# tesseract-robotics/trajopt

Hardware: AMD Instinct MI355X
Metric: SQP iters/s (+ QP solves/s), 7-DOF x 30-wp x 1024-batch glass_upright (higher is better)
Workload: dtype f64; 1 GPU; config 1: glass_upright 7-DOF 30-waypoint, collision cost, batch=1024 random seeds per GPU; n_dof=7, n_steps=30, batch_per_gpu=1024, qp_n=572, qp_m=876, parallelism=seeds sharded, dp1

## Files before the change

### trajopt_amd/csrc/tmx_api.cpp

```cpp
#include <algorithm>
#include <cstddef>
#include <limits>
#include <string>
#include <vector>

#include "tmx_kernels.h"
#include "tmx_wave_kernels.h"
#include "tmx_wave_plan.h"

#ifdef TMX_HOST_EMU
#include <chrono>
thread_local tmx_emu_idx tmx_emu_threadIdx, tmx_emu_blockIdx, tmx_emu_blockDim, tmx_emu_gridDim;
thread_local double* tmx_emu_smem = nullptr;
double tmx_emu_now_ms()
{
  return std::chrono::duration<double, std::milli>(std::chrono::steady_clock::now().time_since_epoch()).count();
}
#else
#include <rccl/rccl.h>
#endif

#define HIPCHK(call)                                                                                                  \
  do                                                                                                                  \
  {                                                                                                                   \
// ... 1528 lines not shown
    int n_coll = 0;
    for (int k : kind)
      n_coll += (k == SLOT_COLLISION || k == SLOT_COLLISION_LVS) ? 1 : 0;
    const char* force = std::getenv("TMX_FORCE_COMPACT");
    const bool on = (force && force[0] == '1') || (!(force && force[0] == '0') && (R >= 1024 || R2 > 0) && 2 * n_coll > R);
    if (on)
      P.coef_far |= 2;
  }
  if (dyn_p && !qp_dense)
    P.coef_far |= 4;
  P.dbg_flags = 0;
  P.wave_ok = 0;
  P.wv_gmax = 2;
  P.wv_aux2 = 0;
  P.wv_plan = nullptr;
  P.row_perm = nullptr;
  {
    const char* env = std::getenv("TMX_ROW_PERM");
    const int NT = TMX_QP_NT;
    if (!(env && env[0] == '0') && R <= 2 * NT && TMX_QP_NT == 256)
    {
      std::vector<int> perm(2 * (size_t)NT, -1), cheap, heavy;
      for (int r = 0; r < R; ++r)
        (naux[r] > 1 ? heavy : cheap).push_back(r);
      const int extra = std::max(0, R - NT), two_first = NT - extra;
      const int prot_first = extra > 0 ? (two_first / 64) * 64 : NT;
      std::vector<int> pool(cheap);
      pool.insert(pool.end(), heavy.begin(), heavy.end());
      size_t take = 0;
      for (int q = 0; q < 2; ++q)
        for (int i = 0; i < extra; ++i)
          perm[(size_t)q * NT + two_first + i] = pool[take++];
      for (int tdx = prot_first; tdx < two_first && take < pool.size(); ++tdx)
        perm[tdx] = pool[take++];
      const int n_free = std::min(prot_first, two_first);
      const size_t n_cheap_left = take < cheap.size() ? cheap.size() - take : 0, n_left = pool.size() - take, n_heavy_left = n_left - n_cheap_left;
      if ((int)n_left > n_free)
        perm.clear();
      else
      {
        for (size_t i = 0; i < n_cheap_left; ++i)
          perm[i] = pool[take + i];
        for (size_t i = 0; i < n_heavy_left; ++i)
          perm[(size_t)n_free - n_heavy_left + i] = pool[take + n_cheap_left + i];
      }
      if (!perm.empty())
      {
        tmx_status rcp;
        if ((rcp = upload(ctx, ctx->prob_allocs, &P.row_perm, perm)) != TMX_OK)
          return rcp;
      }
    }
  }
#if TMX_IS_DEVICE
  {
    const char* env = std::getenv("TMX_WAVE");
    const bool allowed = env && env[0] == '1';
    std::vector<int> plan(TMX_WV_NT * TMX_WV_REC, 0);
    int gmax = 4, aux2 = 0, n3 = 0;
    if (allowed && P.flavor == 0 && R2 == 0 && P.coef_far == 0 && !qp_dense && !P.st && !P.band && !P.use_time && P.n_fx == 0 &&
        wave_plan_build(D, T, R, st.data(), naux.data(), plan.data(), &gmax, &aux2, &n3))
    {
      const size_t small_ints_w = 2 * (size_t)(P.n_max + 1) + 4 * (size_t)R + 2 + 16 + 16 + 512;
      size_t small = std::max<size_t>((tmx_eval_scratch_doubles(R, D * T, (int)vel_first.size(), n_costs, n_cnts) + n_costs + n_cnts + 8) * sizeof(double),
                                      small_ints_w * sizeof(int) + 64);
      small = std::max<size_t>(small, tmx_cvx_scratch_doubles(P.n_cp, D) * sizeof(double));
      const size_t lds = std::max(small, wave_lds_doubles(D, T, R) * sizeof(double));
      if (lds <= 40 * 1024)
      {
        tmx_status rcw;
        if ((rcw = upload(ctx, ctx->prob_allocs, &P.wv_plan, plan)) != TMX_OK)
          return rcw;
        P.wave_ok = 1;
        P.wv_gmax = gmax;
        P.wv_aux2 = aux2;
        ctx->smem_wave = lds;
      }
    }
  }
#endif
  ctx->smem_qp = qp_smem_bytes(D, T, R, NA, R2, P.coef_far);
  ctx->tt_scratch = 0;
  if (P.tt_chain > 0 || P.tv_chain)
  {
    const size_t tt_bytes = ((P.tv_chain ? qp_tv_doubles(D, T) : qp_tt_doubles(D, T, P.tt_chain)) + 2) * sizeof(double);
    const char* force = std::getenv("TMX_TT_PLACE");
    if (TMX_QP_COLD_IN_LDS && !(force && force[0] == '2') && (ctx->smem_qp > 160 * 1024 || ctx->smem_qp + tt_bytes <= 160 * 1024))
    {
      P.tt_place = 1;
      ctx->smem_qp += tt_bytes;
    }
    else
    {
      P.tt_place = 2;
      ctx->tt_scratch = tt_bytes / sizeof(double);
    }
  }
  if (!ctx->dp)
  {
    void* p = nullptr;
    HIPCHK(hipMalloc(&p, sizeof(DevProblem)));
    ctx->dp = static_cast<DevProblem*>(p);
  }
  HIPCHK(hipMemcpy(ctx->dp, &P, sizeof(DevProblem), hipMemcpyHostToDevice));
  if (std::getenv("TMX_VERBOSE"))
    std::fprintf(stderr, "[tmx] QP engine: %s; TotalTime terms %d, as rank-one terms on the block chain %d; squared velocity-with-time cost instances %d, "
// ... 1374 lines not shown
{
  if (!ctx || !a || !b || !out || n < 1 || op < 0 || op > 2)
    return TMX_ERR_INVALID;
  HIPCHK(hipSetDevice(ctx->device));
  std::vector<void*> pool;
  double *da = nullptr, *db = nullptr, *dout = nullptr;
  tmx_status rc;
  if ((rc = dalloc(ctx, pool, &da, (size_t)n)) != TMX_OK || (rc = dalloc(ctx, pool, &db, (size_t)n)) != TMX_OK ||
      (rc = dalloc(ctx, pool, &dout, (size_t)n)) != TMX_OK)
  {
    free_pool(pool);
    return rc;
  }
  hipError_t e = hipMemcpy(da, a, sizeof(double) * n, hipMemcpyHostToDevice);
  if (e == hipSuccess)
    e = hipMemcpy(db, b, sizeof(double) * n, hipMemcpyHostToDevice);
  if (e == hipSuccess)
  {
    TMX_LAUNCH(k_detmath, 64, 256, 0, ctx->stream, op, n, da, db, dout);
    e = hipStreamSynchronize(ctx->stream);
  }
  if (e == hipSuccess)
    e = hipMemcpy(out, dout, sizeof(double) * n, hipMemcpyDeviceToHost);
  free_pool(pool);
  if (e != hipSuccess)
  {
    ctx->err = std::string("tmx_debug_detmath: ") + hipGetErrorString(e);
    return TMX_ERR_DEVICE;
  }
  return TMX_OK;
}

__attribute__((visibility("default"))) tmx_status tmx_debug_admm_iters(tmx_ctx* ctx, int64_t* out)
{
  if (!ctx || !out || ctx->hb.B <= 0)
    return TMX_ERR_INVALID;
  static_assert(sizeof(long long) == sizeof(int64_t), "");
  if (hipMemcpy(out, ctx->hb.admm_iters, sizeof(int64_t) * ctx->hb.B, hipMemcpyDeviceToHost) != hipSuccess)
    return TMX_ERR_DEVICE;
  return TMX_OK;
}

__attribute__((visibility("default"))) tmx_status tmx_debug_set_flags(tmx_ctx* ctx, int flags)
{
  if (!ctx || !ctx->have_problem || !ctx->dp)
    return TMX_ERR_INVALID;
  TMX_REFUSE_WHILE_PENDING(ctx);
  HIPCHK(hipSetDevice(ctx->device));
  ctx->hp.dbg_flags = flags;
  HIPCHK(hipMemcpy(reinterpret_cast<char*>(ctx->dp) + offsetof(DevProblem, dbg_flags), &flags, sizeof(int), hipMemcpyHostToDevice));
  return TMX_OK;
}

__attribute__((visibility("default"))) tmx_status tmx_debug_set_fused(tmx_ctx* ctx, int mode)
{
  if (!ctx || mode < 0 || mode > 2)
    return TMX_ERR_INVALID;
  ctx->mode = mode;
  return TMX_OK;
}

tmx_status tmx_kernel_stats_reset(tmx_ctx* ctx)
{
  if (!ctx)
    return TMX_ERR_INVALID;
  ctx->ms_admm = ctx->ms_convexify = ctx->ms_evaluate = 0.0;
  ctx->launches_admm = 0;
  return TMX_OK;
}
}
```

### trajopt_amd/csrc/tmx_solve.h

```cpp
#pragma once
#include "tmx_qp.h"
#include "tmx_terms.h"

#if TMX_IS_DEVICE
#define TMX_ATOMIC_ADD_U64(ptr, v) atomicAdd((unsigned long long*)(ptr), (unsigned long long)(v))
#else
#define TMX_ATOMIC_ADD_U64(ptr, v) __atomic_fetch_add((unsigned long long*)(ptr), (unsigned long long)(v), __ATOMIC_RELAXED)
#endif

TMX_DEVFN double aux_cost(const DevProblem* P, const double* merit, int r)
{
  if (P->flavor == 1)
  {
    const double cf = (P->slot_kind[r] == SLOT_COLLISION_LVS) ? P->slot_objc[r] : P->slot_scale[r];
    return (P->slot_iscnt[r] ? merit[P->slot_owner[r]] : 1.0) * cf;
  }
  return P->slot_iscnt[r] ? merit[P->slot_owner[r]] : P->slot_objc[r];
}
TMX_DEVFN double primary_q(const DevProblem* P, const double* qdyn, int v)
{
  if (P->flavor == 1)
    return (fabs(qdyn[v]) < 1e-7) ? 0.0 : qdyn[v];
  return P->pq[v];
}

TMX_DEVFN double aux_sign(int naux, int k) { return (naux == 1) ? -1.0 : (k == 0 ? 1.0 : -1.0); }

struct CscOut
{
  long long *P_p, *P_i, *A_p, *A_i;
  double *P_x, *q, *A_x, *l, *u;
};

TMX_DEVFN double tv_p_val(const DevProblem* P, const double* tv_aff, int sgm, int jj, int ia, int ib, bool& any)
{
  double v = 0.0;
  any = false;
  if (tv_aff == nullptr || sgm < 0 || sgm >= P->T - 1)
    return v;
  for (int c = 0; c < P->n_tv; ++c)
    if ((jj < 0 || P->tv_joint[c] == jj) && sgm >= P->tv_first[c] && sgm < P->tv_last[c])
    {
      const double* rec = tv_aff + ((size_t)c * P->T + sgm) * TMX_TV_REC;
      for (int half = 0; half < 2; ++half)
      {
        const double ca = half ? -rec[ia] : rec[ia], cb = half ? -rec[ib] : rec[ib];
        const double coeff = ((ia == ib) ? ca * ca : 2 * ca * cb) * P->tv_coeff[c];
        if (coeff != 0.0)
        {
          v += (ia == ib) ? 2.0 * coeff : coeff;
          any = true;
        }
      }
    }
// ... 882 lines not shown
#ifdef TMX_PROFILE
#define TMX_PROF_ENTER(sh)                                                                                            \
  long long pc[16] = { 0, 0, 0, 0, 0, 0, 0, 0, 0, 0, 0, 0, 0, 0, 0, 0 };                                             \
  long long tlast = TMX_CLK()
#define TMX_PROF_LEAVE(sh)                                                                                            \
  do                                                                                                                  \
  {                                                                                                                   \
    if (threadIdx.x == TMX_PROF_TID)                                                                                  \
      for (int q_ = 0; q_ < 16; ++q_)                                                                                 \
      {                                                                                                               \
        Bt->prof[(size_t)b * 16 + q_] += pc[q_];                                                                      \
        pc[q_] = 0;                                                                                                   \
      }                                                                                                               \
  } while (0)
#else
#define TMX_PROF_ENTER(sh)                                                                                            \
  long long pc[16];                                                                                                   \
  long long tlast = 0;                                                                                                \
  (void)pc;                                                                                                           \
  (void)tlast
#define TMX_PROF_LEAVE(sh) ((void)0)
#endif
TMX_DEVFN QpShared* qp_ws_rebuild(QpWs& w, const DevProblem* P, const DevBatch* Bt, int b, double* smem)
{
  const int D = P->D, T = P->T, R = P->R;
  double* scratch = Bt->qp_scratch + (size_t)b * Bt->qp_scratch_stride;
#if TMX_QP_COLD_IN_LDS
  qp_ws_carve(w, smem, smem + qp_lds_doubles(D, T, R, P->NA, P->n_link), scratch, D, T, R, P->NA, P->n_link, P->coef_far);
#else
  qp_ws_carve(w, smem, scratch + qp_far_doubles(D, T, R, P->NA, P->n_link, P->coef_far), scratch, D, T, R, P->NA, P->n_link, P->coef_far);
#endif
#if TMX_LINK_ROWS
  w.c2i = P->slot_c2;
#endif
  DPart dpt;
  dpart_make(T, dpt);
  qp_ws_alias_deltas(w, P, dpt);
  QpShared* sh = reinterpret_cast<QpShared*>(w.wself);
  w.rho = sh->rho;
  w.sigma = sh->sigma;
  w.alpha = sh->alpha;
  w.c = sh->c;
  w.cinv = sh->cinv;
  return sh;
}
static_assert(sizeof(QpShared) <= sizeof(QpWs), "QpShared must fit the descriptor slot");
template <class T>
TMX_DEVFN T* tmx_uniform_ptr(T* p)
{
  const unsigned long long v = (unsigned long long)p;
  const unsigned lo = __builtin_amdgcn_readfirstlane((unsigned)v), hi = __builtin_amdgcn_readfirstlane((unsigned)(v >> 32));
  return (T*)(((unsigned long long)hi << 32) | lo);
}
__device__ __attribute__((noinline)) static int qp_check_nl(const DevProblem* P_in, const DevBatch* Bt_in, int b_in, int iter_in, unsigned lds_in)
{
  const DevProblem* P = tmx_uniform_ptr(P_in);
  const DevBatch* Bt = tmx_uniform_ptr(Bt_in);
  const int b = __builtin_amdgcn_readfirstlane(b_in), iter = __builtin_amdgcn_readfirstlane(iter_in);
  const int tid = threadIdx.x, NT = TMX_QP_NT;
  double* smem = (double*)(tmx_lds_d*)(size_t)(unsigned)__builtin_amdgcn_readfirstlane((int)lds_in);
  const tmx_osqp_settings& st = P->osqp;
  QpWs w;
  QpShared* sh = qp_ws_rebuild(w, P, Bt, b, smem);
  QpInfo info = sh->info;
  TMX_PROF_ENTER(sh);
  const bool can_check = st.check_termination && (iter % st.check_termination == 0);
  const bool do_rho = st.adaptive_rho && st.adaptive_rho_interval && (iter % st.adaptive_rho_interval == 0);
  int ended = 0;
  if (can_check || do_rho)
  {
    info.iter = iter;
    if (sh->have_res)
    {
      const double* m = sh->res;
      info.prim_res = m[0];
      info.dual_res = w.cinv * m[6];
      info.s_prim = m[1];
      info.s_z = m[2];
      info.s_ax = m[3];
      info.u_z = m[4];
      info.u_ax = m[5];
      info.s_dual = m[7];
      info.s_q = m[8];
      info.s_aty = m[9];
      info.s_px = m[10];
      info.u_q = m[11];
      info.u_aty = m[12];
      info.u_px = m[13];
    }
    else
      compute_residuals(w, P, w.xp, w.xa, w.yr, w.ybp, w.yba, 0, info, info.prim_res, info.dual_res, true, tid, NT);
    TMX_TICK(6);
  }
  if (can_check && TMX_UNI_B(check_termination(w, P, info, false, tid, NT)))
    ended = 1;
  TMX_TICK(3);
  double rho = w.rho;
  if (!ended && do_rho)
  {
    const double rho_new = rho_estimate(w, info);
    if (TMX_UNI_B((rho_new > w.rho * st.adaptive_rho_tolerance) || (rho_new < w.rho / st.adaptive_rho_tolerance)))
    {
      w.rho = fmin(fmax(rho_new, TMX_RHO_MIN), TMX_RHO_MAX);
      rho = w.rho;
      info.rho_updates += 1;
      TMX_TICK(6);
// ... 223 lines not shown
    sh->can_check = can_check ? 1 : 0;
    sh->iter = iter;
#ifdef TMX_PROFILE
    for (int q_ = 0; q_ < 16; ++q_)
      Bt->prof[(size_t)b * 16 + q_] += pc[q_];
#endif
  }
  TMX_SYNC();
}
#endif

template <bool HBM = false, bool BANDK = true, bool ROWSK = true>
TMX_DEVFN void qp_solve_block(const DevProblem* P, const DevBatch* Bt, int b, double* smem, int tid, int NT, double* chain_lds = nullptr)
{
  const int D = P->D, T = P->T, NX = P->NX, R = P->R;
  const tmx_osqp_settings& st = P->osqp;
  QpWs w;
  {
    double* scratch = Bt->qp_scratch + (size_t)b * Bt->qp_scratch_stride;
#if TMX_QP_COLD_IN_LDS
    qp_ws_carve(w, smem, smem + qp_lds_doubles(D, T, R, P->NA, P->n_link), scratch, D, T, R, P->NA, P->n_link, P->coef_far);
#else
    qp_ws_carve(w, smem, scratch + qp_far_doubles(D, T, R, P->NA, P->n_link, P->coef_far), scratch, D, T, R, P->NA, P->n_link, P->coef_far);
#endif
    if (chain_lds)
      qp_ws_chain_to_lds(w, chain_lds);
  }
  if constexpr (BANDK)
    qp_ws_attach_band(w, P->band, Bt->band_ws + (size_t)b * (size_t)Bt->band_stride, (ROWSK && P->band_rows) ? P->n_link : 0);
  [[maybe_unused]] const double* dyn_H = nullptr;
  [[maybe_unused]] const double* dyn_g = nullptr;
  if constexpr (ROWSK)
    if (P->coef_far & 4)
    {
      w.pb = Bt->qp_scratch + (size_t)b * Bt->qp_scratch_stride + qp_dynp_offset(D, T, R, P->NA, P->n_link, P->coef_far);
      dyn_H = Bt->fx_H + (size_t)b * P->n_fx_cost * D * D;
      dyn_g = Bt->fx_g + (size_t)b * P->n_fx_cost * D;
    }
  if constexpr (ROWSK)
    if (P->tt_chain > 0 || P->tv_chain)
      qp_ws_attach_tt(w, P, smem, Bt->qp_scratch + (size_t)b * Bt->qp_scratch_stride);
  long long pc[16] = { 0, 0, 0, 0, 0, 0, 0, 0, 0, 0, 0, 0, 0, 0, 0, 0 };
  long long tlast = TMX_CLK();
  const int* g_act = Bt->active + (size_t)b * R;
  const double* g_coef = Bt->coef + (size_t)b * R * D;
  const double* g_rhs = Bt->rhs + (size_t)b * R;
  [[maybe_unused]] const double* g_coef2 = Bt->coef2 + (size_t)b * P->n_link * D;
  const double* g_x = Bt->x + (size_t)b * NX;
  const double* g_merit = Bt->merit + (size_t)b * P->n_cnts;
  const double trust = Bt->trust[b];
  const int* dims = Bt->dims + 4 * b;
  const unsigned long long* hs = Bt->hashes + 4 * b;

  for (int r = tid; r < R; r += NT)
  {
    w.act[r] = g_act[r];
    w.naux[r] = P->slot_naux[r];
    w.aoff[r] = P->slot_aoff[r];
    w.slot_t[r] = P->slot_t[r];
    w.wp_list[r] = P->wp_list[r];
    w.flg_r[r] = 0;
    w.Er[r] = 1.0;
    w.zr[r] = 0.0;
    w.yr[r] = 0.0;
    w.dyr[r] = 0.0;
    w.lor[r] = P->slot_eq[r] ? g_rhs[r] : -TMX_OSQP_INFTY;
    w.hir[r] = g_rhs[r];
    if (g_act[r] || w.c_alist == nullptr)
    {
      for (int j = 0; j < D; ++j)
        w.coef[r * D + j] = g_act[r] ? g_coef[r * D + j] : 0.0;
#if TMX_LINK_ROWS
      if (P->n_link > 0 && P->slot_c2[r] >= 0)
        for (int j = 0; j < D; ++j)
          w.c2[P->slot_c2[r] * D + j] = g_act[r] ? g_coef2[P->slot_c2[r] * D + j] : 0.0;
#endif
    }
#if TMX_LINK_ROWS
    if (w.band_rows && P->slot_c2[r] >= 0)
    {
      const int ci = P->slot_c2[r];
      const int ord = slot_is_diff(P->slot_kind[r]) ? diff_row_order(P, r) : 1;
      ws_fo(w)[ci] = ord >= 2 ? (ord << 8 | P->slot_sub[r]) : 0;
      ws_cf(w)[2 * ci] = (ord >= 2 && g_act[r]) ? diff_row_coef(P, r, 2) : 0.0;
      ws_cf(w)[2 * ci + 1] = (ord >= 3 && g_act[r]) ? diff_row_coef(P, r, 3) : 0.0;
    }
#endif
    const double oc = aux_cost(P, g_merit, r);
    for (int k = 0; k < P->slot_naux[r]; ++k)
    {
      const int a = P->slot_aoff[r] + k;
      w.sa[a] = aux_sign(P->slot_naux[r], k);
      w.qa[a] = oc;
      w.bba[a] = 1.0;
      w.Da[a] = 1.0;
      w.Eba[a] = 1.0;
      w.xa[a] = 0.0;
      w.zba[a] = 0.0;
      w.yba[a] = 0.0;
      w.dxa[a] = 0.0;
      w.dyba[a] = 0.0;
      w.flg_ba[a] = 0;
    }
  }
  for (int v = tid; v < NX; v += NT)
  {
    const int j = v % D;
    const double xi = fmin(fmax(g_x[v], P->jl[j]), P->ju[j]);
    const double lb = fmax(xi - trust, P->jl[j]), ub = fmin(xi + trust, P->ju[j]);
// ... 52 lines not shown
        bool any;
        double va = 0.0, vc = 0.0;
        if (j < D - 1)
        {
          w.pd[v] = P->pd[v] + tv_p_diag(P, aff, t, j, any);
          if (v < NX - D)
          {
            w.po[v] = P->po[v] + tv_p_val(P, aff, t, j, 0, 1, any);
            vc = tv_p_val(P, aff, t, j, 0, 2, any);
          }
          if (t >= 1)
            va = tv_p_val(P, aff, t - 1, j, 1, 2, any);
        }
        else if (t >= 1)
          w.pd[v] = P->pd[v] + tv_p_val(P, aff, t - 1, -1, 2, 2, any);
        ws_tva(w)[v] = va;
        ws_tvc(w)[v] = vc;
        w.qp[v] = tv_q_lin(P, aff, t, j, w.qp[v]);
      }
    if (w.band)
    {
      w.po2[v] = (v < NX - 2 * D) ? P->po2[v] : 0.0;
      w.po3[v] = (v < NX - 3 * D) ? P->po3[v] : 0.0;
    }
    w.bbp[v] = 1.0;
    w.Dp[v] = 1.0;
    w.Ebp[v] = 1.0;
    w.xp[v] = 0.0;
    w.zbp[v] = 0.0;
    w.ybp[v] = 0.0;
    w.dxp[v] = 0.0;
    w.dybp[v] = 0.0;
    w.flg_bp[v] = 0;
  }
  if constexpr (ROWSK)
    if (w.pb != nullptr)
      for (int e = tid; e < T * D * D; e += NT)
      {
        const int t = e / (D * D), i = (e / D) % D, j = e % D;
        double v = 0.0;
        if (i != j)
          for (int c = 0; c < P->n_fx; ++c)
            if (fx_is_quad(P->fx_kind[c]) && P->fx_t[c] == t)
            {
              const double h = dyn_H[(size_t)P->fx_ci[c] * D * D + (i < j ? i : j) * D + (i < j ? j : i)];
              if (h != 0.0)
                v += h;
            }
        w.pb[e] = v;
      }
  for (int t = tid; t <= T; t += NT)
  {
    w.wp_start[t] = P->wp_start[t];
    int acc = 0;
    for (int u = 0; u < t; ++u)
    {
      const int c = P->wp_start[u + 1] - P->wp_start[u];
      acc += c + (c & 1);
    }
    w.wp_pst[t] = acc;
    for (int u = P->wp_start[t]; t < T && u < P->wp_start[t + 1]; ++u)
      w.row_epos[P->wp_list[u]] = acc + (u - P->wp_start[t]);
  }
#if TMX_LINK_ROWS
  w.c2i = P->slot_c2;
#endif
  w.sigma = st.sigma;
  w.alpha = st.alpha;
  w.c = 1.0;
  w.cinv = 1.0;
  TMX_SYNC();
  {
    int* scan = reinterpret_cast<int*>(w.red);
    const int C = (R + NT - 1) / NT;
    const int r0 = tid * C < R ? tid * C : R, r1 = (tid + 1) * C < R ? (tid + 1) * C : R;
    for (int pass = 0; pass < 2; ++pass)
    {
      int cnt = 0;
      for (int r = r0; r < r1; ++r)
        cnt += w.act[r] ? (pass == 0 ? 1 : w.naux[r]) : 0;
      TMX_SYNC();
      scan[tid] = cnt;
      TMX_SYNC();
      int off = 0;
      for (int u = 0; u < tid; ++u)
        off += scan[u];
      for (int r = r0; r < r1; ++r)
      {
        if (pass == 0)
          w.row_ref[r] = off;
        else
          w.aux_ref[r] = NX + off;
        off += w.act[r] ? (pass == 0 ? 1 : w.naux[r]) : 0;
      }
    }
    TMX_SYNC();
    rows_compact_build(w, P, scan, tid, NT);
  }
  const int n = dims[0], m = dims[1], mg = m - n;
  DPart dpt;
  dpart_make(T, dpt);
  const bool lds_tmp = (w.G != nullptr) && ((size_t)NX + 3 * (size_t)P->NA <= (size_t)dpt.P * w.Gn * w.Gs);
  double* const t_ebp = lds_tmp ? w.G : w.dybp;
  double* const t_eba = lds_tmp ? w.G + NX : w.dyba;
  double* const t_da = lds_tmp ? w.G + NX + P->NA : w.ta;
  double* const acc_da = lds_tmp ? w.G + NX + 2 * P->NA : w.Da;
  if (lds_tmp)
  {
    for (int a = tid; a < P->NA; a += NT)
      acc_da[a] = 1.0;
    TMX_SYNC();
  }

#if defined(TMX_FINE) && TMX_FINE == 4
  TMX_TICK(13);
#endif
  for (int it = 0; it < st.scaling; ++it)
  {
    for (int v = tid; v < NX; v += NT)
    {
      const int t = v / D, j = v % D;
      double cn = fabs(w.pd[v]);
      if (t > 0)
        cn = fmax(cn, fabs(w.po[v - D]));
      if (t < T - 1)
        cn = fmax(cn, fabs(w.po[v]));
      if (w.band)
        cn = fmax(cn, band_col_norm(w, v));
      if (w.pb != nullptr)
        for (int i = 0; i < D; ++i)
          cn = fmax(cn, fabs(w.pb[(size_t)t * D * D + i * D + j]));
      if (w.tvo != 0)
        cn = fmax(cn, tv_p_col_norm(w, v));
      {
        const int q1 = w.wl_start[t + 1];
        int q = w.wl_start[t];
        for (; q + 4 <= q1; q += 4)
        {
          const int r0 = w.wl_list[q], r1 = w.wl_list[q + 1], r2 = w.wl_list[q + 2], r3 = w.wl_list[q + 3];
          const int a0 = w.act[r0], a1 = w.act[r1], a2 = w.act[r2], a3 = w.act[r3];
          const double c0 = w.coef[r0 * D + j], c1 = w.coef[r1 * D + j], c2 = w.coef[r2 * D + j], c3 = w.coef[r3 * D + j];
          cn = a0 ? fmax(cn, fabs(c0)) : cn;
          cn = a1 ? fmax(cn, fabs(c1)) : cn;
          cn = a2 ? fmax(cn, fabs(c2)) : cn;
          cn = a3 ? fmax(cn, fabs(c3)) : cn;
        }
        for (; q < q1; ++q)
        {
          const int r = w.wl_list[q];
          if (w.act[r])
            cn = fmax(cn, fabs(w.coef[r * D + j]));
        }
      }
#if TMX_LINK_ROWS
      if (w.n_link > 0 && t > 0)
        for (int q = w.wl_start[t - 1]; q < w.wl_start[t]; ++q)
        {
          const int r = w.wl_list[q];
          if (w.act[r] && w.c2i[r] >= 0)
            cn = fmax(cn, fabs(w.c2[w.c2i[r] * D + j]));
        }
      if (w.band_rows)
        for (int k = 2; k <= 3 && k <= t; ++k)
          for (int q = w.wl_start[t - k]; q < w.wl_start[t - k + 1]; ++q)
          {
            const int r = w.wl_list[q];
            const int ci = w.c2i[r];
            if (!w.act[r] || ci < 0)
              continue;
// ... 161 lines not shown
      c_temp = limit_scaling(c_temp);
      w.red[128] = 1.0 / c_temp;
    }
    TMX_SYNC();
    const double ct = w.red[128];
    for (int v = tid; v < NX; v += NT)
    {
      w.pd[v] *= ct;
      w.po[v] *= ct;
      if (w.band)
      {
        w.po2[v] *= ct;
        w.po3[v] *= ct;
      }
      w.qp[v] *= ct;
    }
    if (w.pb != nullptr)
      for (int e = tid; e < T * D * D; e += NT)
        w.pb[e] *= ct;
    if (w.ttn > 0 && tid == 0)
      for (int k = 0; k < w.ttn; ++k)
        ws_ttw(w)[k] *= ct;
    if (w.tvo != 0)
      for (int v = tid; v < 2 * NX; v += NT)
        ws_tva(w)[v] *= ct;
    TMX_ROWS(w, r)
      if (w.act[r])
        for (int k = 0; k < w.naux[r]; ++k)
          w.qa[w.aoff[r] + k] *= ct;
    w.c *= ct;
    TMX_SYNC();
  }
  w.cinv = 1.0 / w.c;
  if (lds_tmp)
    for (int a = tid; a < P->NA; a += NT)
      w.Da[a] = acc_da[a];
  for (int v = tid; v < NX; v += NT)
  {
    w.lbp[v] *= w.Ebp[v];
    w.ubp[v] *= w.Ebp[v];
    w.typ_bp[v] = constr_type(w.lbp[v], w.ubp[v]);
  }
  TMX_ROWS(w, r)
  {
    if (!w.act[r])
      continue;
    w.lor[r] *= w.Er[r];
    w.hir[r] *= w.Er[r];
    w.typ_r[r] = constr_type(w.lor[r], w.hir[r]);
    for (int k = 0; k < w.naux[r]; ++k)
      w.typ_ba[w.aoff[r] + k] = constr_type(0.0, TMX_OSQP_INFTY * w.Eba[w.aoff[r] + k]);
  }
  TMX_SYNC();

#if defined(TMX_FINE) && TMX_FINE == 4
  TMX_TICK(15);
#endif
  const int* pd4 = Bt->prev_dims + 4 * b;
  const unsigned long long* pws = Bt->prev_ws + 2 * b;
  bool warm = Bt->prev_ok[b] && st.warm_starting;
  const bool P_eq = warm && pd4[0] == dims[0] && pd4[2] == dims[2] && pws[0] == hs[2];
  const bool A_eq = P_eq && pd4[0] == dims[0] && pd4[1] == dims[1] && pd4[3] == dims[3] && pws[1] == hs[3];
  warm = TMX_UNI_B(warm && P_eq && A_eq);
#if defined(TMX_HOST_EMU) && !defined(TMX_EMU_SIMT)
  if (const char* fq = std::getenv("TMX_EMU_FAULT_WARM_QP"))
    if (Bt->rec_count[b] >= std::atoi(fq) && warm)
      warm = false;
#endif
  if (P->flavor == 1)
  {
    warm = TMX_UNI_B(st.warm_starting != 0);
    w.rho = Bt->prev_ok[b] ? Bt->prev_rho[b] : st.rho;
  }
  else
    w.rho = warm ? Bt->prev_rho[b] : st.rho;
  w.rho = fmin(fmax(w.rho, TMX_RHO_MIN), TMX_RHO_MAX);
  if (warm)
  {
    const double* xq = Bt->xq + (size_t)b * P->n_max;
    const double* yq = Bt->yq + (size_t)b * P->m_max;
    for (int v = tid; v < NX; v += NT)
    {
      w.xp[v] = (1.0 / w.Dp[v]) * xq[v];
      w.ybp[v] = ((1.0 / w.Ebp[v]) * yq[mg + v]) * w.c;
    }
    TMX_ROWS(w, r)
      if (w.act[r])
      {
        w.yr[r] = ((1.0 / w.Er[r]) * yq[w.row_ref[r]]) * w.c;
        for (int k = 0; k < w.naux[r]; ++k)
        {
          const int a = w.aoff[r] + k;
          w.xa[a] = (1.0 / w.Da[a]) * xq[w.aux_ref[r] + k];
          w.yba[a] = ((1.0 / w.Eba[a]) * yq[mg + w.aux_ref[r] + k]) * w.c;
        }
      }
    TMX_SYNC();
    for (int v = tid; v < NX; v += NT)
      w.zbp[v] = w.bbp[v] * w.xp[v];
    TMX_ROWS(w, r)
      if (w.act[r])
      {
        const int t = w.slot_t[r];
        double ax = 0.0;
        for (int j = 0; j < D; ++j)
          ax += w.coef[r * D + j] * w.xp[t * D + j];
#if TMX_LINK_ROWS
        ax += link_dot(w, r, t, w.xp);
#endif
        for (int k = 0; k < w.naux[r]; ++k)
        {
          const int a = w.aoff[r] + k;
          ax += w.sa[a] * w.xa[a];
          w.zba[a] = w.bba[a] * w.xa[a];
        }
        w.zr[r] = ax;
      }
    TMX_SYNC();
  }

  TMX_TICK(0);
#if TMX_IS_DEVICE
  const bool fast = TMX_UNI_B(!HBM && (NT == TMX_QP_NT) && (R <= 512) && dpart_supported(w, NT) && !TMX_HAS_PAIRS(w) && w.c_alist == nullptr && w.band == 0 && w.pb == nullptr && w.ttn == 0 && w.tvo == 0 && TMX_FAST_ALLOWED);
#else
  const bool fast = false;
#endif
#if TMX_IS_DEVICE
  if (fast)
    qp_ws_alias_deltas(w, P, dpt);
#endif
  kkt_factor(w, P, 0, w.sigma, st.delta, tid, NT);
  kkt_invert(w, fast, tid, NT, pc, tlast);
  if (w.ttn > 0)
    tt_factor(w, tid, NT);
  admm_cache_weights(w, tid, NT);
  TMX_TICK(15);
  QpInfo info;
  info.status = 11;
  info.iter = 0;
  info.rho_updates = 0;
  info.polish_status = 0;
  info.prim_res = info.dual_res = 0.0;
  int iter = 0;
  bool can_check = false, terminated = false;
#if TMX_ADMM_OUTLINED
  if (fast)
  {
    QpShared* sh = reinterpret_cast<QpShared*>(w.wself);
    if (tid == 0)
    {
      sh->rho = w.rho;
      sh->sigma = w.sigma;
      sh->alpha = w.alpha;
      sh->c = w.c;
      sh->cinv = w.cinv;
      sh->info = info;
      sh->terminated = 0;
      sh->can_check = 0;
      sh->iter = 0;
      sh->have_res = 0;
    }
    TMX_SYNC();
    {
      unsigned lds_off = (unsigned)(size_t)smem;
      TMX_ASM_OPAQUE_SGPR(lds_off);
      qp_admm_fast_nl(P, Bt, b, lds_off);
    }
#ifdef TMX_PROFILE
    tlast = TMX_CLK();
#endif
    info = sh->info;
    w.rho = sh->rho;
    terminated = sh->terminated != 0;
    can_check = sh->can_check != 0;
    iter = sh->iter;
    TMX_SYNC();
  }
  else
#endif
// ... 1234 lines not shown
```

### trajopt_amd/csrc/tmx_types.h

```cpp
#pragma once
#include "../../include/tmx.h"
#include "tmx_platform.h"

enum
{
  SLOT_FIXED = 0,
  SLOT_CARTPOSE = 1,
  SLOT_JOINTPOS = 2,
  SLOT_COLLISION = 3,
  SLOT_JOINTPOS_INEQ = 4,
  SLOT_JOINTVEL = 5,
  SLOT_JOINTVEL_INEQ = 6,
  SLOT_COLLISION_LVS = 7,
  SLOT_FUNC = 9,
  SLOT_CARTVEL = 8,
  SLOT_JOINTVEL_TIME = 10,
  SLOT_TOTAL_TIME = 11
};
#ifndef TMX_LINK_ROWS
#define TMX_LINK_ROWS 1
#endif

enum
{
// ... 23 lines not shown
  int *wp_list;
  double *pd, *po, *pq;
  int *p_colptr;
  int *vel_first, *vel_last, *vel_cost, *vel_kind;
  double *vel_coeffs, *vel_targets;
  int *cp_t, *cp_owner, *cp_iscnt, *cp_nrows, *cp_idx, *cp_slot0;
  double *cp_coeff, *cp_target;
  int *ls_link;
  double *ls_center, *ls_radius, *ob_center, *ob_radius;
  int *own_lo, *own_hi;
  int coef_far;
  double *ob_axis;
  int *slot_c2;
  int n_link;
  int *slot_sub3;
  double *slot_aux3;
  int lvs_kmax;
  int flavor;
  int n_sq;
  double *po2, *po3;
  int n_stencil;
  int qp_dense;
  int st;
  int n_fx, n_fx_cost;
  int *fx_t, *fx_kind, *fx_owner, *fx_op0, *fx_nops, *fx_c0, *fx_nout, *fx_slot0, *fx_ci;
  int *fx_ops;
  double *fx_consts;
  double *ls_axis;
  int n_ls_capsule;
  double *ob_box;
  int n_ob_box;
  double *mesh;
  int band;
  int band_rows;
  int* ls_hull;
  double* hull;
  int n_ls_hull;
  int DK;
  int use_time;
  int n_tv;
  int *tv_owner, *tv_joint, *tv_first, *tv_last;
  double *tv_coeff, *tv_target, *tv_up, *tv_lo;
  int n_tt;
  int *tt_owner, *tt_form, *tt_slot;
  double *tt_coeff, *tt_limit;
  int wave_ok;
  int wv_gmax;
  int wv_aux2;
  int* wv_plan;
  int* row_perm;
  int dbg_flags;
  int tt_chain, tt_place;
  int tv_chain;
};
TMX_HOSTDEVFN int slot_is_diff(int kind) { return kind == SLOT_JOINTVEL || kind == SLOT_JOINTVEL_INEQ; }
#define TMX_TV_REC 5
TMX_HOSTDEVFN int fx_is_quad(int kind) { return kind == 0 || kind == 1 || kind == 3; }
TMX_HOSTDEVFN int fx_is_rows(int kind) { return kind == 2 || kind == 4; }

struct DevBatch
{
  int B, max_rec;
  double *x0, *x, *xnew;
  double *cost_vals, *cnt_viols, *new_cost_vals, *new_cnt_viols, *merit;
  double *trust, *total_cost, *prev_rho;
  int *phase, *iter, *merit_inc, *qp_fail, *status, *retval, *n_fe, *n_qp, *cvx, *prev_ok;
  int *active;
  double *coef, *rhs;
  double *qdyn;
  double *rowc;
  int *solver_init;
  double *coef2;
  int *dims;
  unsigned long long *hashes;
  int *prev_dims;
  unsigned long long *prev_ws;
  double *xq, *yq;
  tmx_qp_record *rec_last, *rec_log;
  int *rec_count;
  long long *admm_iters;
  int *n_active;
  int *sched_state;
  int *sched_done;
  int *tail_flag;
  double *qp_scratch;
  long long qp_scratch_stride;
  long long *prof;
  double *ws_hbm;
  long long ws_hbm_stride;
  int ws_chain_in_lds;
  double *step_log;
  int step_log_stride;
  int *accept_flag;
  long long *t_start;
  long long *dq_Pp, *dq_Pi, *dq_Ap, *dq_Ai;
  double *dq_Px, *dq_Ax, *dq_q, *dq_l, *dq_u;
  double *dq_x, *dq_y, *dq_xw, *dq_yw;
  int *dq_flags;
  double *dq_ws;
  long long dq_ws_stride;
  int dq_nnzA;
  int dq_nnzP;
  tmx_qp_info* dq_info;
  double *fx_H, *fx_g, *fx_c, *fx_W;
  double *band_ws;
  long long band_stride;
  double *tv_aff, *tt_aff;
};

#ifndef TMX_ADMM_OUTLINED
#if defined(TMX_BURST_NOINLINE) || defined(TMX_HOST_EMU)
#define TMX_ADMM_OUTLINED 0
#else
#define TMX_ADMM_OUTLINED 1
#endif
#endif
```

Before: 152,700 SQP iters/s.

## Add register-resident fast Ruiz equilibration path for QP setup

Adds a fast setup path that keeps each thread's variable column and up to two constraint rows in registers across Ruiz scaling passes. Row norms are exchanged through a small LDS array indexed by precomputed per-waypoint positions uploaded from the host. The per-thread prefix scan for active-row offsets is replaced with a wave ballot/popcount scan. The goal is to cut the LDS traffic, barriers and serial scan loop in QP setup. The trade-offs are higher register pressure and a path restricted by row-count and aux limits. Note that the wp_pst, row_epos and hr fields used in QpWs are not visible being carved, so the change may be incomplete.

Measured after the change: 160,400 SQP iters/s (median of 6 runs). 1.05x the previous value.

```diff
diff --git a/trajopt_amd/csrc/tmx_api.cpp b/trajopt_amd/csrc/tmx_api.cpp
--- a/trajopt_amd/csrc/tmx_api.cpp
+++ b/trajopt_amd/csrc/tmx_api.cpp
@@ -1604,6 +1604,29 @@
       }
     }
   }
+  P.wp_pst = P.row_epos = nullptr;
+  P.setup_fast = 0;
+  {
+    std::vector<int> pst(T + 1, 0), epos(R, 0);
+    int acc = 0, rows_max = 0, naux_max = 0;
+    for (int t = 0; t <= T; ++t)
+    {
+      pst[t] = acc;
+      if (t == T)
+        break;
+      const int c = wp_start[t + 1] - wp_start[t];
+      for (int u = wp_start[t]; u < wp_start[t + 1]; ++u)
+        epos[wp_list[u]] = acc + (u - wp_start[t]);
+      acc += c + (c & 1);
+      rows_max = std::max(rows_max, c);
+    }
+    for (int r = 0; r < R; ++r)
+      naux_max = std::max(naux_max, naux[r]);
+    tmx_status rcs;
+    if ((rcs = upload(ctx, ctx->prob_allocs, &P.wp_pst, pst)) != TMX_OK || (rcs = upload(ctx, ctx->prob_allocs, &P.row_epos, epos)) != TMX_OK)
+      return rcs;
+    P.setup_fast = (rows_max <= TMX_SETUP_COL && naux_max <= 2 && R <= 2 * TMX_QP_NT) ? 1 : 0;
+  }
 #if TMX_IS_DEVICE
   {
     const char* env = std::getenv("TMX_WAVE");
@@ -3084,6 +3107,13 @@
   return TMX_OK;
 }
 
+__attribute__((visibility("default"))) int tmx_debug_setup_fast(tmx_ctx* ctx)
+{
+  if (!ctx || !ctx->have_problem)
+    return -1;
+  return ctx->hp.setup_fast;
+}
+
 __attribute__((visibility("default"))) tmx_status tmx_debug_set_fused(tmx_ctx* ctx, int mode)
 {
   if (!ctx || mode < 0 || mode > 2)
diff --git a/trajopt_amd/csrc/tmx_setup.h b/trajopt_amd/csrc/tmx_setup.h
--- /dev/null
+++ b/trajopt_amd/csrc/tmx_setup.h
@@ -0,0 +1,228 @@
+#pragma once
+#include "tmx_qp.h"
+
+#if TMX_IS_DEVICE
+struct SetupRow
+{
+  int r, t, na, ao, epos;
+  bool on;
+  double c[8], sa[2], bba[2], qa[2], Da[2], Eba[2], Er;
+};
+
+TMX_DEVFN double ruiz_fast(const QpWs& w, const DevProblem* P, int n_pass, int n, int tid)
+{
+  constexpr int NT = TMX_QP_NT;
+  const int D = w.D, T = w.T, NX = w.NX, R = w.R;
+  for (int e = tid; e < T * 8; e += NT)
+    w.tp[e] = 0.0;
+  for (int e = tid; e < R + T + TMX_SETUP_COL; e += NT)
+    w.hr[e] = 0.0;
+  SetupRow g[2];
+  {
+    const int* rperm = P->row_perm;
+#pragma unroll
+    for (int q = 0; q < 2; ++q)
+    {
+      SetupRow& s = g[q];
+      const int slot = q * NT + tid;
+      s.r = rperm ? rperm[slot] : (slot < R ? slot : -1);
+      s.on = s.r >= 0 && s.r < R && w.act[s.r >= 0 && s.r < R ? s.r : 0] != 0;
+      const int r = s.on ? s.r : 0;
+      s.t = w.slot_t[r];
+      s.na = s.on ? w.naux[r] : 0;
+      s.ao = w.aoff[r];
+      s.epos = w.row_epos[r];
+#pragma unroll
+      for (int j = 0; j < 8; ++j)
+        s.c[j] = (s.on && j < D) ? w.coef[r * D + j] : 0.0;
+#pragma unroll
+      for (int k = 0; k < 2; ++k)
+      {
+        const bool ok = k < s.na;
+        s.sa[k] = ok ? w.sa[s.ao + k] : 0.0;
+        s.qa[k] = ok ? w.qa[s.ao + k] : 0.0;
+        s.bba[k] = ok ? w.bba[s.ao + k] : 0.0;
+        s.Da[k] = 1.0;
+        s.Eba[k] = 1.0;
+      }
+      s.Er = 1.0;
+    }
+  }
+  const bool pv = tid < NX;
+  const int v = pv ? tid : 0, vt = v / D, vj = v - vt * D;
+  const bool has_prev = pv && vt > 0, has_next = pv && vt < T - 1;
+  double pd = pv ? w.pd[v] : 0.0, po = pv ? w.po[v] : 0.0, pop = has_prev ? w.po[v - D] : 0.0;
+  double bbp = pv ? w.bbp[v] : 0.0, qp = pv ? w.qp[v] : 0.0, Dp = 1.0, Ebp = 1.0;
+  double cj[TMX_SETUP_COL];
+  const int e0 = w.wp_pst[vt];
+  {
+    const int q0 = w.wp_start[vt], q1 = w.wp_start[vt + 1];
+#pragma unroll
+    for (int k = 0; k < TMX_SETUP_COL; ++k)
+    {
+      const bool ok = pv && q0 + k < q1;
+      const int r = ok ? w.wp_list[q0 + k] : 0;
+      cj[k] = ok ? w.coef[r * D + vj] : 0.0;
+    }
+  }
+  double c_run = 1.0;
+  TMX_SYNC();
+  for (int it = 0; it < n_pass; ++it)
+  {
+    double dv = 0.0, ebp = 0.0;
+    if (pv)
+    {
+      double cn = fabs(pd);
+      if (has_prev)
+        cn = fmax(cn, fabs(pop));
+      if (has_next)
+        cn = fmax(cn, fabs(po));
+#pragma unroll
+      for (int k = 0; k < TMX_SETUP_COL; ++k)
+        cn = fmax(cn, fabs(cj[k]));
+      cn = fmax(cn, fabs(bbp));
+      dv = 1.0 / sqrt(limit_scaling(cn));
+      ebp = 1.0 / sqrt(limit_scaling(fabs(bbp)));
+      w.tp[vt * 8 + vj] = dv;
+    }
+    double er[2] = { 0.0, 0.0 }, da[2][2] = { { 0.0, 0.0 }, { 0.0, 0.0 } }, eba[2][2] = { { 0.0, 0.0 }, { 0.0, 0.0 } };
+#pragma unroll
+    for (int q = 0; q < 2; ++q)
+      if (g[q].on)
+      {
+        SetupRow& s = g[q];
+        double rn = 0.0;
+#pragma unroll
+        for (int j = 0; j < 8; ++j)
+          rn = fmax(rn, fabs(s.c[j]));
+#pragma unroll
+        for (int k = 0; k < 2; ++k)
+          if (k < s.na)
+          {
+            rn = fmax(rn, fabs(s.sa[k]));
+            da[q][k] = 1.0 / sqrt(limit_scaling(fmax(fabs(s.sa[k]), fabs(s.bba[k]))));
+            eba[q][k] = 1.0 / sqrt(limit_scaling(fabs(s.bba[k])));
+          }
+        er[q] = 1.0 / sqrt(limit_scaling(rn));
+        w.hr[s.epos] = er[q];
+      }
+    TMX_SYNC();
+    if (pv)
+    {
+      const double dn = has_next ? w.tp[(vt + 1) * 8 + vj] : 0.0, dl = has_prev ? w.tp[(vt - 1) * 8 + vj] : 0.0;
+      pd = (dv * pd) * dv;
+      if (has_next)
+        po = (dv * po) * dn;
+      if (has_prev)
+        pop = (dl * pop) * dv;
+      bbp = (ebp * bbp) * dv;
+      qp *= dv;
+      Dp *= dv;
+      Ebp *= ebp;
+#pragma unroll
+      for (int k = 0; k < TMX_SETUP_COL; ++k)
+        cj[k] = (w.hr[e0 + k] * cj[k]) * dv;
+    }
+#pragma unroll
+    for (int q = 0; q < 2; ++q)
+      if (g[q].on)
+      {
+        SetupRow& s = g[q];
+#pragma unroll
+        for (int j = 0; j < 8; ++j)
+          s.c[j] = (er[q] * s.c[j]) * w.tp[s.t * 8 + j];
+#pragma unroll
+        for (int k = 0; k < 2; ++k)
+          if (k < s.na)
+          {
+            s.sa[k] = (er[q] * s.sa[k]) * da[q][k];
+            s.bba[k] = (eba[q][k] * s.bba[k]) * da[q][k];
+            s.qa[k] *= da[q][k];
+            s.Da[k] *= da[q][k];
+            s.Eba[k] *= eba[q][k];
+          }
+        s.Er *= er[q];
+      }
+    double nrm[2] = { 0.0, 0.0 };
+    if (pv)
+    {
+      double cn = fabs(pd);
+      if (has_prev)
+        cn = fmax(cn, fabs(pop));
+      if (has_next)
+        cn = fmax(cn, fabs(po));
+      nrm[1] = cn;
+      nrm[0] = fabs(qp);
+    }
+#pragma unroll
+    for (int q = 0; q < 2; ++q)
+      if (g[q].on)
+      {
+#pragma unroll
+        for (int k = 0; k < 2; ++k)
+          if (k < g[q].na)
+            nrm[0] = fmax(nrm[0], fabs(g[q].qa[k]));
+      }
+    {
+      const bool issum[2] = { false, true };
+      block_reduce<2>(nrm, issum, w.red, tid, NT);
+    }
+    double c_temp = nrm[1] / (double)n;
+    c_temp = fmax(c_temp, limit_scaling(nrm[0]));
+    c_temp = limit_scaling(c_temp);
+    const double ct = 1.0 / c_temp;
+    pd *= ct;
+    po *= ct;
+    pop *= ct;
+    qp *= ct;
+#pragma unroll
+    for (int q = 0; q < 2; ++q)
+#pragma unroll
+      for (int k = 0; k < 2; ++k)
+        g[q].qa[k] *= ct;
+    c_run *= ct;
+  }
+  if (pv)
+  {
+    w.pd[v] = pd;
+    w.po[v] = po;
+    w.bbp[v] = bbp;
+    w.qp[v] = qp;
+    w.Dp[v] = Dp;
+    w.Ebp[v] = Ebp;
+    const double lb = w.lbp[v] * Ebp, ub = w.ubp[v] * Ebp;
+    w.lbp[v] = lb;
+    w.ubp[v] = ub;
+    w.typ_bp[v] = constr_type(lb, ub);
+  }
+#pragma unroll
+  for (int q = 0; q < 2; ++q)
+    if (g[q].on)
+    {
+      const SetupRow& s = g[q];
+#pragma unroll
+      for (int j = 0; j < 8; ++j)
+        if (j < D)
+          w.coef[s.r * D + j] = s.c[j];
+#pragma unroll
+      for (int k = 0; k < 2; ++k)
+        if (k < s.na)
+        {
+          const int a = s.ao + k;
+          w.sa[a] = s.sa[k];
+          w.bba[a] = s.bba[k];
+          w.qa[a] = s.qa[k];
+          w.Da[a] = s.Da[k];
+          w.Eba[a] = s.Eba[k];
+          w.typ_ba[a] = constr_type(0.0, TMX_OSQP_INFTY * s.Eba[k]);
+        }
+      w.Er[s.r] = s.Er;
+      const double lo = w.lor[s.r] * s.Er, hi = w.hir[s.r] * s.Er;
+      w.lor[s.r] = lo;
+      w.hir[s.r] = hi;
+      w.typ_r[s.r] = constr_type(lo, hi);
+    }
+  TMX_SYNC();
+  return c_run;
+}
+#endif
diff --git a/trajopt_amd/csrc/tmx_solve.h b/trajopt_amd/csrc/tmx_solve.h
--- a/trajopt_amd/csrc/tmx_solve.h
+++ b/trajopt_amd/csrc/tmx_solve.h
@@ -1,5 +1,6 @@
 #pragma once
 #include "tmx_qp.h"
+#include "tmx_setup.h"
 #include "tmx_terms.h"
 
 #if TMX_IS_DEVICE
@@ -988,6 +989,28 @@
   const unsigned lo = __builtin_amdgcn_readfirstlane((unsigned)v), hi = __builtin_amdgcn_readfirstlane((unsigned)(v >> 32));
   return (T*)(((unsigned long long)hi << 32) | lo);
 }
+#ifndef TMX_SETUP_OUTLINED
+#define TMX_SETUP_OUTLINED 1
+#endif
+#if TMX_SETUP_OUTLINED
+__device__ __attribute__((noinline)) static double qp_ruiz_fast_nl(const DevProblem* P_in, const DevBatch* Bt_in, int b_in, unsigned lds_in)
+{
+  const DevProblem* P = tmx_uniform_ptr(P_in);
+  const DevBatch* Bt = tmx_uniform_ptr(Bt_in);
+  const int b = __builtin_amdgcn_readfirstlane(b_in);
+  const int tid = threadIdx.x;
+  double* smem = (double*)(tmx_lds_d*)(size_t)(unsigned)__builtin_amdgcn_readfirstlane((int)lds_in);
+  const int D = P->D, T = P->T, R = P->R;
+  double* scratch = Bt->qp_scratch + (size_t)b * Bt->qp_scratch_stride;
+  QpWs w;
+#if TMX_QP_COLD_IN_LDS
+  qp_ws_carve(w, smem, smem + qp_lds_doubles(D, T, R, P->NA, P->n_link), scratch, D, T, R, P->NA, P->n_link, P->coef_far);
+#else
+  qp_ws_carve(w, smem, scratch + qp_far_doubles(D, T, R, P->NA, P->n_link, P->coef_far), scratch, D, T, R, P->NA, P->n_link, P->coef_far);
+#endif
+  return ruiz_fast(w, P, P->osqp.scaling, Bt->dims[4 * b], tid);
+}
+#endif
 __device__ __attribute__((noinline)) static int qp_check_nl(const DevProblem* P_in, const DevBatch* Bt_in, int b_in, int iter_in, unsigned lds_in)
 {
   const DevProblem* P = tmx_uniform_ptr(P_in);
@@ -1317,9 +1340,18 @@
   const int* dims = Bt->dims + 4 * b;
   const unsigned long long* hs = Bt->hashes + 4 * b;
 
+#if TMX_IS_DEVICE
+  const bool fast = TMX_UNI_B(!HBM && (NT == TMX_QP_NT) && (R <= 512) && dpart_supported(w, NT) && !TMX_HAS_PAIRS(w) && w.c_alist == nullptr && w.band == 0 && w.pb == nullptr && w.ttn == 0 && w.tvo == 0 && TMX_FAST_ALLOWED);
+  const bool fast_setup = TMX_UNI_B(fast && P->setup_fast != 0 && !(P->dbg_flags & 2));
+#else
+  const bool fast = false;
+  const bool fast_setup = false;
+#endif
   for (int r = tid; r < R; r += NT)
   {
     w.act[r] = g_act[r];
+    if (fast_setup)
+      w.row_epos[r] = P->row_epos[r];
     w.naux[r] = P->slot_naux[r];
     w.aoff[r] = P->slot_aoff[r];
     w.slot_t[r] = P->slot_t[r];
@@ -1478,6 +1510,11 @@
   for (int t = tid; t <= T; t += NT)
   {
     w.wp_start[t] = P->wp_start[t];
+    if (fast_setup)
+    {
+      w.wp_pst[t] = P->wp_pst[t];
+      continue;
+    }
     int acc = 0;
     for (int u = 0; u < t; ++u)
     {
@@ -1505,12 +1542,35 @@
       int cnt = 0;
       for (int r = r0; r < r1; ++r)
         cnt += w.act[r] ? (pass == 0 ? 1 : w.naux[r]) : 0;
-      TMX_SYNC();
-      scan[tid] = cnt;
-      TMX_SYNC();
       int off = 0;
-      for (int u = 0; u < tid; ++u)
-        off += scan[u];
+#if TMX_IS_DEVICE
+      if (fast_setup)
+      {
+        const int lane = tid & 63, wave = tid >> 6;
+        const unsigned long long below = (1ull << lane) - 1ull;
+        int tot = 0;
+        for (int bit = 0; bit < 3; ++bit)
+        {
+          const unsigned long long mk = __builtin_amdgcn_ballot_w64(((cnt >> bit) & 1) != 0);
+          off += __builtin_popcountll(mk & below) << bit;
+          tot += __builtin_popcountll(mk) << bit;
+        }
+        TMX_SYNC();
+        if (lane == 0)
+          scan[wave] = tot;
+        TMX_SYNC();
+        for (int u = 0; u < wave; ++u)
+          off += scan[u];
+      }
+      else
+#endif
+      {
+        TMX_SYNC();
+        scan[tid] = cnt;
+        TMX_SYNC();
+        for (int u = 0; u < tid; ++u)
+          off += scan[u];
+      }
       for (int r = r0; r < r1; ++r)
       {
         if (pass == 0)
@@ -1531,7 +1591,7 @@
   double* const t_eba = lds_tmp ? w.G + NX : w.dyba;
   double* const t_da = lds_tmp ? w.G + NX + P->NA : w.ta;
   double* const acc_da = lds_tmp ? w.G + NX + 2 * P->NA : w.Da;
-  if (lds_tmp)
+  if (lds_tmp && !fast_setup)
   {
     for (int a = tid; a < P->NA; a += NT)
       acc_da[a] = 1.0;
@@ -1541,6 +1601,21 @@
 #if defined(TMX_FINE) && TMX_FINE == 4
   TMX_TICK(13);
 #endif
+#if TMX_IS_DEVICE
+  if (fast_setup)
+  {
+#if TMX_ADMM_OUTLINED && TMX_SETUP_OUTLINED
+    unsigned lds_off = (unsigned)(size_t)smem;
+    TMX_ASM_OPAQUE_SGPR(lds_off);
+    w.c = qp_ruiz_fast_nl(P, Bt, b, lds_off);
+#else
+    w.c = ruiz_fast(w, P, st.scaling, n, tid);
+#endif
+    w.cinv = 1.0 / w.c;
+  }
+  else
+#endif
+  {
   for (int it = 0; it < st.scaling; ++it)
   {
     for (int v = tid; v < NX; v += NT)
@@ -1808,6 +1883,7 @@
       w.typ_ba[w.aoff[r] + k] = constr_type(0.0, TMX_OSQP_INFTY * w.Eba[w.aoff[r] + k]);
   }
   TMX_SYNC();
+  }
 
 #if defined(TMX_FINE) && TMX_FINE == 4
   TMX_TICK(15);
@@ -1876,11 +1952,6 @@
   }
 
   TMX_TICK(0);
-#if TMX_IS_DEVICE
-  const bool fast = TMX_UNI_B(!HBM && (NT == TMX_QP_NT) && (R <= 512) && dpart_supported(w, NT) && !TMX_HAS_PAIRS(w) && w.c_alist == nullptr && w.band == 0 && w.pb == nullptr && w.ttn == 0 && w.tvo == 0 && TMX_FAST_ALLOWED);
-#else
-  const bool fast = false;
-#endif
 #if TMX_IS_DEVICE
   if (fast)
     qp_ws_alias_deltas(w, P, dpt);
diff --git a/trajopt_amd/csrc/tmx_types.h b/trajopt_amd/csrc/tmx_types.h
--- a/trajopt_amd/csrc/tmx_types.h
+++ b/trajopt_amd/csrc/tmx_types.h
@@ -99,6 +99,8 @@
   int dbg_flags;
   int tt_chain, tt_place;
   int tv_chain;
+  int *wp_pst, *row_epos;
+  int setup_fast;
 };
 TMX_HOSTDEVFN int slot_is_diff(int kind) { return kind == SLOT_JOINTVEL || kind == SLOT_JOINTVEL_INEQ; }
 #define TMX_TV_REC 5
@@ -155,6 +157,7 @@
   double *tv_aff, *tt_aff;
 };
 
+#define TMX_SETUP_COL 18
 #ifndef TMX_ADMM_OUTLINED
 #if defined(TMX_BURST_NOINLINE) || defined(TMX_HOST_EMU)
 #define TMX_ADMM_OUTLINED 0
```
